# RIVM-bioinformatics/TrueConsense

Measured on AMD Instinct MI355X. Metric: reference positions/sec (BAM file -> consensus FASTA, 1M reads x 29 903 bp per BAM), higher is better.
Workload: dtype int32

## Files before the change

### trueconsense_amd/csrc/bgzf_device.h

```cpp
#pragma once
#include "bgzf_host.h"
#include "tcmi_internal.h"

namespace {

#ifndef TCMI_INFLATE_LL_ROOT
#define TCMI_INFLATE_LL_ROOT 9
#endif
#ifndef TCMI_INFLATE_D_ROOT
#define TCMI_INFLATE_D_ROOT 8
#endif
constexpr int LL_ROOT = TCMI_INFLATE_LL_ROOT, D_ROOT = TCMI_INFLATE_D_ROOT, CL_ROOT = 7;
static_assert(D_ROOT >= CL_ROOT, "the code-length table borrows the distance table's LDS");
constexpr int MAX_REC_PER_BLOCK = 65536 / 36 + 2;

static __constant__ uint8_t CL_ORDER[19] = {16, 17, 18, 0, 8, 7, 9, 6, 10, 5, 11, 4, 12, 3, 13, 2, 14, 1, 15};

__device__ inline uint32_t uni(uint32_t v) { return (uint32_t)__builtin_amdgcn_readfirstlane((int)v); }
__device__ __forceinline__ void wave_sync() { __builtin_amdgcn_fence(__ATOMIC_ACQ_REL, "wavefront"); __builtin_amdgcn_wave_barrier(); }

template <int CTRL, int ROW_MASK>
__device__ __forceinline__ uint32_t dpp_shift(uint32_t v)
{
    return (uint32_t)__builtin_amdgcn_update_dpp(0, (int)v, CTRL, ROW_MASK, 0xF, true);
}
__device__ __forceinline__ uint32_t wave_scan_add(uint32_t v)
{
    v += dpp_shift<0x111, 0xF>(v);
    v += dpp_shift<0x112, 0xF>(v);
    v += dpp_shift<0x114, 0xF>(v);
    v += dpp_shift<0x118, 0xF>(v);
    v += dpp_shift<0x142, 0xA>(v);
    v += dpp_shift<0x143, 0xC>(v);
    return v;
}
__device__ __forceinline__ uint32_t wave_scan_max(uint32_t v)
{
    v = max(v, dpp_shift<0x111, 0xF>(v));
    v = max(v, dpp_shift<0x112, 0xF>(v));
    v = max(v, dpp_shift<0x114, 0xF>(v));
    v = max(v, dpp_shift<0x118, 0xF>(v));
    v = max(v, dpp_shift<0x142, 0xA>(v));
    v = max(v, dpp_shift<0x143, 0xC>(v));
    return v;
}

constexpr uint32_t E_LIT = 1u << 8, E_BASE = 1u << 9, E_EOB = 1u << 10;
enum { K_LITLEN = 0, K_DIST = 1, K_CODELEN = 2 };

typedef uint32_t tab_t;

__device__ inline uint32_t make_entry(int kind, int sym, int nbits)
{
    if (sym < 0) return 0u;
    if (kind == K_CODELEN) return (uint32_t)nbits | ((uint32_t)sym << 16);
    if (kind == K_LITLEN) {
        if (sym < 256) return (uint32_t)nbits | E_LIT | ((uint32_t)sym << 16);
        if (sym == 256) return (uint32_t)nbits | E_EOB;
        const int s = sym - 257;
        if (s > 28) return 0u;
        int eb = 0, base = 3 + s;
        if (s == 28) base = 258;
        else if (s >= 8) { eb = (s >> 2) - 1; base = 3 + ((4 + (s & 3)) << eb); }
        return (uint32_t)nbits | ((uint32_t)(nbits + eb) << 11) | E_BASE | ((uint32_t)eb << 16) | ((uint32_t)base << 20);
    }
    if (sym > 29) return 0u;
    int eb = 0, base = 1 + sym;
    if (sym >= 4) { eb = (sym >> 1) - 1; base = 1 + ((2 + (sym & 1)) << eb); }
    return (uint32_t)nbits | ((uint32_t)eb << 4) | E_BASE | ((uint32_t)base << 16);
}

template <int MAXG, int ROOT>
__device__ __forceinline__ bool build_table(const uint8_t *lens, int n, uint16_t *cnt, uint16_t *sym, tab_t *tab, int kind, uint32_t *rs)
{
    const int lane = threadIdx.x & 63;
    wave_sync();
    int l[MAXG];
#pragma unroll
    for (int g = 0; g < MAXG; ++g) l[g] = g * 64 + lane < n ? (int)lens[g * 64 + lane] : 0;
    int c[16];
#pragma unroll
    for (int len = 0; len < 16; ++len) c[len] = 0;
#pragma unroll
    for (int g = 0; g < MAXG; ++g) {
#pragma unroll
        for (int len = 1; len <= 15; ++len) c[len] += (int)__popcll(__ballot(l[g] == len));
    }
    {
        int mine = 0;
#pragma unroll
        for (int len = 1; len <= 15; ++len) mine = lane == len ? c[len] : mine;
        if (lane < 16) cnt[lane] = (uint16_t)mine;
    }
    int off[16], first[16];
    int left = 1, o = 0, f = 0;
    bool ok = true;
#pragma unroll
    for (int len = 1; len <= 15; ++len) {
        left = (left << 1) - c[len];
        if (left < 0) ok = false;
        off[len] = o;
        first[len] = f;
        o += c[len];
        f = (f + c[len]) << 1;
        if (len == ROOT && lane == 0) { rs[0] = (uint32_t)f; rs[1] = (uint32_t)o; }
    }
    {
        int nx[16];
#pragma unroll
        for (int len = 1; len <= 15; ++len) nx[len] = off[len];
#pragma unroll
        for (int g = 0; g < MAXG; ++g) {
#pragma unroll
            for (int len = 1; len <= 15; ++len) {
                const unsigned long long m = __ballot(l[g] == len);
                if (m) {
                    const int below = (int)__builtin_amdgcn_mbcnt_hi((uint32_t)(m >> 32), __builtin_amdgcn_mbcnt_lo((uint32_t)m, 0u));
                    if (l[g] == len) sym[nx[len] + below] = (uint16_t)(g * 64 + lane);
                    nx[len] += (int)__popcll(m);
                }
            }
        }
    }
    wave_sync();
    for (int i = lane; i < (1 << ROOT); i += 64) {
        const uint32_t r = __builtin_bitreverse32((uint32_t)i) >> (32 - ROOT);
        int L = 0, si = 0;
#pragma unroll
        for (int len = 1; len <= ROOT; ++len) {
            const uint32_t d = (r >> (ROOT - len)) - (uint32_t)first[len];
            const bool hit = d < (uint32_t)c[len];
            L = hit ? len : L;
            si = hit ? off[len] + (int)d : si;
        }
        tab[i] = L ? make_entry(kind, (int)sym[si], L) : 0u;
    }
    wave_sync();
    return uni(ok ? 1u : 0u) != 0;
}

constexpr uint32_t TOK_LIT = 1u << 31, TOK_RAW = 1u << 30;
constexpr uint32_t TOK_LIT2 = 1u << 24;
constexpr uint32_t RAW_PIECE = 8191;

#define TCMI_STAMP(buf_, blk_, k_) do { if (buf_) { if ((threadIdx.x & 63) == 0) (buf_)[(size_t)(blk_) * 16 + (k_)] = __builtin_amdgcn_s_memtime(); } } while (0)
#define TCMI_STAMP_ADD(buf_, blk_, k_, v_) do { if (buf_) { if ((threadIdx.x & 63) == 0) (buf_)[(size_t)(blk_) * 16 + (k_)] += (v_); } } while (0)

}

struct tcmi_bgzf_decode_args {
    const uint8_t *d_file;
    const void *d_desc;
    uint32_t *d_tok;
    uint32_t *d_ntok;
    uint8_t *d_out;
    uint32_t *d_slot;
    uint32_t *d_nrec;
    int32_t *d_over;
    uint32_t *d_first;
    uint32_t *d_stat;
    size_t n_blocks;
    size_t first_block = 0, count = ~(size_t)0;
    uint64_t tok_base = 0;
    uint32_t pay_dwords;
    uint32_t n_ref;
    int verify_crc = 1;
    int scratch_div = 1;
    int short_tokens;
};
int tcmi_bgzf_decode_launch(tcmi_ctx *ctx, const tcmi_bgzf_decode_args &a);
int tcmi_bgzf_symbols_launch(tcmi_ctx *ctx, const tcmi_bgzf_decode_args &a, size_t b_first, size_t nb, uint64_t *stamps, bool report, bool *two_literals);
int tcmi_bgzf_copy_launch(tcmi_ctx *ctx, const tcmi_bgzf_decode_args &a, size_t b_first, size_t nb, uint64_t *stamps, bool report, bool two_literals);
```

### trueconsense_amd/csrc/bgzf_symbols.hip

```cpp
#include <algorithm>
#include <cstdio>
#include <cstdlib>

#include "bgzf_device.h"

namespace {

constexpr int CL_SLAB = 496;
struct BlkTabs {
    tab_t ll[1 << LL_ROOT];
    tab_t dt[1 << D_ROOT];
    tab_t long_ll[288], long_d[32];
    uint32_t lim_ll[16 - LL_ROOT], fb_ll[16 - LL_ROOT], lim_d[16 - D_ROOT], fb_d[16 - D_ROOT];
    uint32_t pos;
    uint32_t end;
    uint32_t ntok;
    uint32_t err;
    uint32_t go;
    uint32_t last;
};
struct HdrScratch {
    uint8_t lens[320];
    uint8_t cll[20];
    uint16_t sym_ll[288], sym_d[32], sym_cl[20];
    uint16_t cnt_ll[16], cnt_d[16], cnt_cl[16];
    uint32_t rs[6];
};
#ifndef TCMI_SYM_MOVE
#define TCMI_SYM_MOVE 8
#endif
#ifndef TCMI_SYM_ROWS
#define TCMI_SYM_ROWS 32
#endif
#ifndef TCMI_SYM_WAVES
#define TCMI_SYM_WAVES 5
#endif
constexpr int RING = 8;
struct PassALds {
    uint2 ring[64][RING];
    uint2 rec[64];
};
template <int NB>
struct SymLds {
    BlkTabs b[NB];
    union {
        HdrScratch h[NB];
        PassALds a;
    };
};
static_assert((CL_SLAB + 16) * 4 <= sizeof(tab_t) * (1 << LL_ROOT), "the code-length position table borrows the literal/length table's LDS");

struct SymArgs {
    const uint32_t *__restrict__ file32;
    const BlockDesc *blocks;
    uint32_t *tokens;
    uint32_t *n_tok;
    uint32_t *status;
    int32_t n_blocks;
    int32_t first_block;
    uint32_t pay_dwords;
    uint32_t win_dwords;
    uint32_t gather_max;
    uint32_t shift_bias;
    uint32_t scratch_div;
    uint64_t *stamps;
};

__device__ __forceinline__ uint32_t peek32(const uint32_t *pay, uint32_t p)
{
    const uint32_t w = p >> 5;
    return __builtin_amdgcn_alignbit(pay[w + 1], pay[w], p);
}
__device__ __forceinline__ void peek64(const uint32_t *pay, uint32_t p, uint32_t &lo, uint32_t &hi)
{
    const uint32_t w = p >> 5;
    const uint32_t w0 = pay[w], w1 = pay[w + 1], w2 = pay[w + 2];
    lo = __builtin_amdgcn_alignbit(w1, w0, p);
    hi = __builtin_amdgcn_alignbit(w2, w1, p);
}

template <int ROOT>
__device__ __forceinline__ void build_long(const uint16_t *cnt, const uint16_t *sym, const uint32_t *rs, int kind, tab_t *out, uint32_t *lim_out,
                                           uint32_t *fb_out)
{
    const int lane = threadIdx.x & 63;
    uint32_t first = uni(rs[0]);
    const uint32_t at = uni(rs[1]);
    uint32_t n = 0;
    uint32_t cs[15 - ROOT];
    uint32_t my_lim = 0x10000u, my_fb = 0;
#pragma unroll
    for (int len = ROOT + 1; len <= 15; ++len) {
        const uint32_t c = uni(cnt[len]);
        cs[len - ROOT - 1] = c;
        if (lane == len - ROOT - 1) { my_lim = (first + c) << (15 - len); my_fb = (first & 0xFFFFu) | (n << 16); }
        first = (first + c) << 1;
        n += c;
    }
    if (lane <= 15 - ROOT) { lim_out[lane] = my_lim; fb_out[lane] = my_fb; }
    for (uint32_t i = (uint32_t)lane; i < n; i += 64) {
        uint32_t base = 0;
        int mylen = 15;
#pragma unroll
        for (int len = ROOT + 1; len <= 15; ++len) {
            const uint32_t c = cs[len - ROOT - 1];
            if (i >= base && i < base + c) mylen = len;
            base += c;
        }
        out[i] = make_entry(kind, (int)sym[at + i], mylen);
    }
}

template <int ROOT>
__device__ __forceinline__ uint32_t long_lookup(const uint32_t *lim, const uint32_t *fb, const tab_t *tab, uint32_t bits)
{
    const uint32_t r15 = __builtin_bitreverse32(bits) >> 17;
    uint32_t n = 0;
#pragma unroll
    for (int k = 0; k < 15 - ROOT; ++k) n += r15 >= lim[k] ? 1u : 0u;
    if (n >= (uint32_t)(15 - ROOT)) return 0u;
    const uint32_t f = fb[n];
    const uint32_t code = r15 >> (14 - ROOT - n);
    if (code < (f & 0xFFFFu)) return 0u;
    return tab[(f >> 16) + (code - (f & 0xFFFFu))];
}

template <int NB>
__device__ __forceinline__ uint32_t group_scan_add(uint32_t v)
{
    v += dpp_shift<0x111, 0xF>(v);
    v += dpp_shift<0x112, 0xF>(v);
    v += dpp_shift<0x114, 0xF>(v);
    v += dpp_shift<0x118, 0xF>(v);
    v += dpp_shift<0x142, 0xA>(v);
    if (NB == 1) v += dpp_shift<0x143, 0xC>(v);
    return v;
}

enum { SY_LIT = 0, SY_MATCH = 1, SY_EOB = 2, SY_BAD = 3 };

__device__ __forceinline__ void block_header(BlkTabs &T, HdrScratch &H, const uint32_t *pay, uint32_t base_bit, uint32_t *toks, uint32_t cap, bool &last,
                                          uint64_t *stamps, int blk, bool one_header = false)
{
    const int lane = threadIdx.x & 63;
    uint32_t pos = uni(T.pos), ntok = uni(T.ntok), err = ST_OK;
    const uint32_t end = uni(T.end);
    bool go = false;
    while (!last && err == ST_OK && !go) {
        if (pos + 3u > end) { err = ST_BAD_STREAM; break; }
        const uint32_t h = uni(peek32(pay, pos));
        last = (h & 1u) != 0;
        const uint32_t type = (h >> 1) & 3u;
        pos += 3;
        if (type == 0) {
            pos = (pos + 7u) & ~7u;
            if (pos + 32u > end) { err = ST_BAD_STREAM; break; }
            const uint32_t v = uni(peek32(pay, pos));
            const uint32_t len = v & 0xFFFFu;
            if (((v >> 16) ^ len) != 0xFFFFu) { err = ST_BAD_STREAM; break; }
            pos += 32;
            if (pos + len * 8u > end) { err = ST_BAD_STREAM; break; }
            const uint32_t off = (pos - base_bit) >> 3;
            const uint32_t pieces = (len + RAW_PIECE - 1u) / RAW_PIECE;
            if (ntok + pieces > cap) { err = ST_BAD_STREAM; break; }
            if ((uint32_t)lane < pieces) {
                const uint32_t o = (uint32_t)lane * RAW_PIECE;
                toks[ntok + (uint32_t)lane] = TOK_RAW | (min(len - o, RAW_PIECE) << 17) | (off + o);
            }
            ntok += pieces;
            pos += len * 8u;
            if (one_header) break;
            continue;
        }
        if (type == 3) { err = ST_BAD_STREAM; break; }
        int nlen = 288, ndist = 32;
        wave_sync();
        if (type == 1) {
            for (int i = lane; i < 320; i += 64) H.lens[i] = i < 144 ? 8 : i < 256 ? 9 : i < 280 ? 7 : i < 288 ? 8 : 5;
        } else {
            if (pos + 14u > end) { err = ST_BAD_STREAM; break; }
            const uint32_t hh = uni(peek32(pay, pos));
            nlen = (int)(hh & 31u) + 257;
            ndist = (int)((hh >> 5) & 31u) + 1;
            const int ncode = (int)((hh >> 10) & 15u) + 4;
            pos += 14;
            if (nlen > 286 || ndist > 30) { err = ST_BAD_STREAM; break; }
            if (lane < 19) H.cll[lane] = 0;
            wave_sync();
            for (int i0 = 0; i0 < ncode; i0 += 8) {
                const uint32_t v = uni(peek32(pay, pos + (uint32_t)i0 * 3u));
                const int k = i0 + lane;
                if (lane < 8 && k < ncode) H.cll[CL_ORDER[k]] = (uint8_t)((v >> (3 * lane)) & 7u);
            }
            pos += (uint32_t)ncode * 3u;
            if (uni(build_table<1, CL_ROOT>(H.cll, 19, H.cnt_cl, H.sym_cl, T.dt, K_CODELEN, H.rs + 4) ? 1u : 0u) == 0u) { err = ST_BAD_STREAM; break; }
            for (int i = lane; i < 320; i += 64) H.lens[i] = 0;
            uint32_t *const P = T.ll;
            uint32_t got = 0, prev = 0;
            const uint32_t total = (uint32_t)(nlen + ndist);
            bool first = true;
            while (got < total && err == ST_OK) {
                wave_sync();
#pragma unroll 2
                for (int o = lane; o < CL_SLAB + 16; o += 64) {
                    const uint32_t v = peek32(pay, pos + (uint32_t)o);
                    const uint32_t e = T.dt[v & ((1u << CL_ROOT) - 1u)];
                    const uint32_t nb = e & 15u, sym = e >> 16;
                    const uint32_t x = v >> nb;
                    const uint32_t eb = sym < 16u ? 0u : sym == 16u ? 2u : sym == 17u ? 3u : 7u;
                    const uint32_t rep = sym < 16u ? 1u : sym == 18u ? 11u + (x & 127u) : 3u + (x & (sym == 16u ? 3u : 7u));
                    const uint32_t val = sym <= 16u ? sym : 0u;
                    P[o] = nb && o < CL_SLAB ? (nb + eb) | (rep << 4) | (val << 12) : 0u;
                }
                wave_sync();
                uint16_t *const J = reinterpret_cast<uint16_t *>(T.long_ll);
                static_assert(sizeof(T.long_ll) >= 512 * sizeof(uint16_t) && CL_SLAB + 16 <= 512, "the doubling table borrows the long-code table's LDS");
#pragma unroll
                for (int i = 0; i < 8; ++i) {
                    const uint32_t at0 = (uint32_t)lane + 64u * i;
                    const uint32_t e0 = at0 < (uint32_t)CL_SLAB + 16u ? P[at0] : 0u;
                    J[at0] = (uint16_t)(e0 ? at0 + (e0 & 15u) : at0);
                }
                wave_sync();
                uint32_t pm[5];
                pm[0] = 0;
#pragma unroll
                for (int k = 0; k < 6; ++k) {
                    if (((uint32_t)lane >> k) & 1u) pm[0] = J[pm[0]];
                    uint32_t t8[8];
#pragma unroll
                    for (int i = 0; i < 8; ++i) t8[i] = J[lane + 64 * i];
#pragma unroll
                    for (int i = 0; i < 8; ++i) t8[i] = J[t8[i]];
                    wave_sync();
#pragma unroll
                    for (int i = 0; i < 8; ++i) J[lane + 64 * i] = (uint16_t)t8[i];
                    wave_sync();
                }
#pragma unroll
                for (int m = 1; m < 5; ++m) pm[m] = J[pm[m - 1]];
                uint32_t o = 0;
                bool stopped = false;
#pragma unroll
                for (int m = 0; m < 5; ++m) {
                    if (!(got < total && err == ST_OK && !stopped)) break;
                    uint32_t mine = P[pm[m]];
                    const unsigned long long zmask = __ballot(mine == 0);
                    const uint32_t nv = zmask ? (uint32_t)__builtin_ctzll(zmask) : 64u;
                    if ((uint32_t)lane >= nv) mine = 0;
                    uint32_t rep = (mine >> 4) & 255u;
                    const uint32_t incl0 = wave_scan_add(rep);
                    const unsigned long long reach = __ballot(mine != 0 && got + incl0 >= total);
                    const uint32_t n_take = reach ? min(nv, (uint32_t)__builtin_ctzll(reach) + 1u) : nv;
                    if ((uint32_t)lane >= n_take) { mine = 0; rep = 0; }
                    const uint32_t v = mine >> 12;
                    const uint32_t at = got + incl0 - ((mine >> 4) & 255u);
                    const uint32_t named = wave_scan_max(mine != 0 && v != 16u ? (uint32_t)lane + 1u : 0u);
                    const uint32_t theirs = (uint32_t)__builtin_amdgcn_ds_bpermute((int)((named - 1u) << 2), (int)v);
                    const uint32_t val = named ? theirs : prev;
                    if (__ballot(mine != 0 && (at + rep > total || (first && lane == 0 && v == 16u)))) { err = ST_BAD_STREAM; break; }
                    if (mine != 0 && val != 0) {
#pragma unroll
                        for (uint32_t i = 0; i < 6; ++i)
                            if (i < rep) H.lens[at + i] = (uint8_t)val;
                    }
                    if (n_take) {
                        prev = (uint32_t)__builtin_amdgcn_readlane((int)val, (int)(n_take - 1u));
                        got += (uint32_t)__builtin_amdgcn_readlane((int)incl0, (int)(n_take - 1u));
                        o = (uint32_t)__builtin_amdgcn_readlane((int)(pm[m] + (mine & 15u)), (int)(n_take - 1u));
                        first = false;
                    }
                    if (n_take < 64u && got < total) {
                        stopped = true;
                        o = (uint32_t)__builtin_amdgcn_readlane((int)pm[m], (int)n_take);
                        if (o < (uint32_t)CL_SLAB) err = ST_BAD_STREAM;
                    }
                }
                if (err == ST_OK && got < total && !stopped) err = ST_BAD_STREAM;
                pos += o;
                if (pos > end) err = ST_BAD_STREAM;
            }
            if (err != ST_OK) break;
            wave_sync();
            if (uni(H.lens[256]) == 0) { err = ST_BAD_STREAM; break; }
        }
        TCMI_STAMP(stamps, blk, 2);
        if (uni(build_table<5, LL_ROOT>(H.lens, nlen, H.cnt_ll, H.sym_ll, T.ll, K_LITLEN, H.rs) ? 1u : 0u) == 0u) { err = ST_BAD_STREAM; break; }
        if (uni(build_table<1, D_ROOT>(H.lens + nlen, ndist, H.cnt_d, H.sym_d, T.dt, K_DIST, H.rs + 2) ? 1u : 0u) == 0u) { err = ST_BAD_STREAM; break; }
        build_long<LL_ROOT>(H.cnt_ll, H.sym_ll, H.rs, K_LITLEN, T.long_ll, T.lim_ll, T.fb_ll);
        build_long<D_ROOT>(H.cnt_d, H.sym_d, H.rs + 2, K_DIST, T.long_d, T.lim_d, T.fb_d);
        if (pos >= end) { err = ST_BAD_STREAM; break; }
        go = true;
        TCMI_STAMP(stamps, blk, 3);
    }
    wave_sync();
    if (lane == 0) { T.pos = pos; T.ntok = ntok; T.err = err; T.go = go && err == ST_OK ? 1u : 0u; T.last = last ? 1u : 0u; }
}

#define TCMI_PAIR_LOOK "v_lshrrev_b32 v44, v50, v47\n" "v_and_b32 v44, 0x1ff, v44\n" "v_lshl_add_u32 v44, v44, 2, %[tabs]\n" "ds_read_b32 v44, v44\n"
#define TCMI_PAIR_RESOLVE "s_waitcnt lgkmcnt(0)\n" "v_and_b32 v40, v49, v44\n" "v_and_b32 v45, 15, v44\n" "v_add_u32 v46, v52, v45\n" "v_xor_b32 v42, %[p], v52\n" "v_lshrrev_b32 v42, %[shift], v42\n" "v_bfe_u32 v40, v40, 8, 1\n" "v_cmp_gt_u32 vcc, 10, v50\n" "v_cmp_eq_u32 s[86:87], 1, v40\n" "s_and_b64 vcc, vcc, s[86:87]\n" "v_cmp_eq_u32 s[86:87], 0, v42\n" "s_and_b64 vcc, vcc, s[86:87]\n" "v_cmp_le_u32 s[86:87], v46, %[wend]\n" "s_and_b64 vcc, vcc, s[86:87]\n" "v_bfe_u32 v40, v44, 16, 8\n" "v_lshl_or_b32 v40, v40, 8, v51\n" "v_or_b32 v40, 0x1000000, v40\n" "v_cndmask_b32 v51, v51, v40, vcc\n" "v_cndmask_b32 v52, v52, v46, vcc\n"
#define TCMI_PASS_A_ASM(PAIR_LOOK_, PAIR_RESOLVE_) \
                asm volatile( \
                    "s_mov_b64 s[92:93], exec\n" \
                    "LT%=:\n" \
                    "s_mov_b64 exec, %[run]\n" \
                    "s_cbranch_execz LX%=\n" \
                    "v_lshrrev_b32 v40, %[shift], %[p]\n" \
                    "v_cmp_ne_u32 vcc, v40, %[kprev]\n" \
                    "s_and_saveexec_b64 s[80:81], vcc\n" \
                    "s_cbranch_execz LA1%=\n" \
                    "v_mov_b32 %[kprev], v40\n" \
                    "v_and_b32 v41, 7, v40\n" \
                    "v_lshl_add_u32 v41, v41, 3, %[ringb]\n" \
                    "ds_write2_b32 v41, %[p], %[total] offset1:1\n" \
                    "v_mov_b32 %[crossp], %[p]\n" \
                    "v_mov_b32 %[crosst], %[total]\n" \
                    "LA1%=:\n" \
                    "s_mov_b64 exec, %[run]\n" \
                    "s_and_b32 s90, %[rounds], 3\n" \
                    "s_cmp_eq_u32 s90, 3\n" \
                    "s_cbranch_scc0 LC%=\n" \
                    "v_cmp_ne_u32 vcc, -1, %[crossp]\n" \
                    "s_and_saveexec_b64 s[80:81], vcc\n" \
                    "s_cbranch_execz LB9%=\n" \
                    "v_add_u32 v41, -1, %[lim]\n" \
                    "v_min_u32 v41, %[tgt], v41\n" \
                    "v_lshl_add_u32 v42, v41, 3, %[recbase]\n" \
                    "ds_read2_b32 v[44:45], v42 offset1:1\n" \
                    "v_lshrrev_b32 v40, %[shift], %[crossp]\n" \
                    "v_and_b32 v40, 7, v40\n" \
                    "v_lshlrev_b32 v40, 3, v40\n" \
                    "s_waitcnt lgkmcnt(0)\n" \
                    "v_and_b32 v43, 3, v44\n" \
                    "v_cmp_ne_u32 vcc, 0, v43\n" \
                    "v_cmp_ge_u32 s[86:87], %[crossp], v45\n" \
                    "s_and_b64 vcc, vcc, s[86:87]\n" \
                    "v_cmp_lt_u32 s[86:87], %[tgt], %[lim]\n" \
                    "s_and_b64 vcc, vcc, s[86:87]\n" \
                    "s_and_saveexec_b64 s[82:83], vcc\n" \
                    "v_cmp_eq_u32 vcc, 1, v43\n" \
                    "v_add_u32 %[tgt], 1, %[tgt]\n" \
                    "s_and_b64 exec, exec, vcc\n" \
                    "v_lshrrev_b32 %[tgt], 8, v44\n" \
                    "s_mov_b64 exec, s[82:83]\n" \
                    "v_cmp_lt_u32 vcc, %[tgt], %[lim]\n" \
                    "s_and_b64 exec, exec, vcc\n" \
                    "s_cbranch_execz LB8%=\n" \
                    "v_lshl_add_u32 v42, %[tgt], 6, v40\n" \
                    "v_add_u32 v42, %[ringbase], v42\n" \
                    "ds_read2_b32 v[44:45], v42 offset1:1\n" \
                    "s_waitcnt lgkmcnt(0)\n" \
                    "v_cmp_eq_u32 vcc, v44, %[crossp]\n" \
                    "s_and_b64 exec, exec, vcc\n" \
                    "s_cbranch_execz LB8%=\n" \
                    "v_mov_b32 %[midx], v45\n" \
                    "v_mov_b32 %[state], 1\n" \
                    "v_mov_b32 %[p], %[crossp]\n" \
                    "v_mov_b32 %[total], %[crosst]\n" \
                    "v_lshl_or_b32 v43, %[tgt], 8, 1\n" \
                    "ds_write2_b32 %[recb], v43, %[p] offset1:1\n" \
                    "s_andn2_b64 %[run], %[run], exec\n" \
                    "LB8%=:\n" \
                    "s_mov_b64 exec, s[80:81]\n" \
                    "v_mov_b32 %[crossp], -1\n" \
                    "LB9%=:\n" \
                    "s_mov_b64 exec, %[run]\n" \
                    "s_cbranch_execz LX%=\n" \
                    "LC%=:\n" \
                    "v_cmp_lt_u32 vcc, %[p], %[wend]\n" \
                    "s_xor_b64 s[86:87], vcc, exec\n" \
                    "s_cmp_lg_u64 s[86:87], 0\n" \
                    "s_cbranch_scc1 LDend%=\n" \
                    "LC1%=:\n" \
                    "v_lshrrev_b32 v40, 5, %[p]\n" \
                    "v_lshl_add_u32 v40, v40, 2, %[pay]\n" \
                    "ds_read2_b32 v[44:45], v40 offset1:1\n" \
                    "ds_read_b32 v46, v40 offset:8\n" \
                    "s_waitcnt lgkmcnt(0)\n" \
                    "v_alignbit_b32 v47, v45, v44, %[p]\n" \
                    "v_alignbit_b32 v48, v46, v45, %[p]\n" \
                    "v_and_b32 v40, 0x1ff, v47\n" \
                    "v_lshl_add_u32 v40, v40, 2, %[tabs]\n" \
                    "ds_read_b32 v49, v40\n" \
                    "s_waitcnt lgkmcnt(0)\n" \
                    "v_and_b32 v50, 15, v49\n" \
                    "v_cmp_eq_u32 vcc, 0, v50\n" \
                    "s_cbranch_vccnz LLl%=\n" \
                    "LC2%=:\n" \
                    "v_bfe_u32 v41, v49, 8, 3\n" \
                    "v_cmp_eq_u32 vcc, 4, v41\n" \
                    "s_cbranch_vccnz LDeob%=\n" \
                    "LC3%=:\n" \
                    "v_bfe_u32 v51, v49, 16, 8\n" \
                    "v_or_b32 v51, 0x80000000, v51\n" \
                    "v_add_u32 v52, %[p], v50\n" \
                    PAIR_LOOK_ \
                    "s_mov_b64 s[88:89], exec\n" \
                    "v_cmp_eq_u32 vcc, 2, v41\n" \
                    "s_and_b64 exec, exec, vcc\n" \
                    "s_cbranch_execz LC5%=\n" \
                    "v_bfe_u32 v53, v49, 11, 5\n" \
                    "v_alignbit_b32 v54, v48, v47, v53\n" \
                    "v_and_b32 v40, 0xff, v54\n" \
                    "v_lshl_add_u32 v40, v40, 2, %[tabs]\n" \
                    "ds_read_b32 v55, v40 offset:%[odt]\n" \
                    "v_lshrrev_b32 v42, v50, v47\n" \
                    "v_bfe_u32 v43, v49, 16, 4\n" \
                    "v_bfe_u32 v42, v42, 0, v43\n" \
                    "v_bfe_u32 v43, v49, 20, 9\n" \
                    "v_add_u32 v56, v43, v42\n" \
                    "s_waitcnt lgkmcnt(0)\n" \
                    "v_and_b32 v57, 15, v55\n" \
                    "v_cmp_eq_u32 vcc, 0, v57\n" \
                    "s_cbranch_vccnz LLd%=\n" \
                    "LC4%=:\n" \
                    "v_bfe_u32 v43, v55, 4, 4\n" \
                    "v_lshrrev_b32 v42, v57, v54\n" \
                    "v_bfe_u32 v42, v42, 0, v43\n" \
                    "v_lshrrev_b32 v40, 16, v55\n" \
                    "v_add_u32 v42, v42, v40\n" \
                    "v_add_u32 v42, -1, v42\n" \
                    "v_lshl_or_b32 v51, v42, 9, v56\n" \
                    "v_add3_u32 v52, %[p], v53, v57\n" \
                    "v_add_u32 v52, v52, v43\n" \
                    "LC5%=:\n" \
                    "s_and_b64 exec, s[88:89], %[run]\n" \
                    "s_cbranch_execz LT%=\n" \
                    PAIR_RESOLVE_ \
                    "v_mov_b32 %[p], v52\n" \
                    "v_cmp_gt_u32 vcc, %[p], %[end]\n" \
                    "s_cbranch_vccnz LDover%=\n" \
                    "LC6%=:\n" \
                    "s_mov_b64 s[80:81], exec\n" \
                    "v_cmp_ne_u32 vcc, 0, %[room]\n" \
                    "s_and_b64 exec, exec, vcc\n" \
                    "global_store_dword %[sptr], v51, off\n" \
                    "v_add_u32 %[room], -1, %[room]\n" \
                    "v_lshl_add_u64 %[sptr], %[sptr], 0, %[sstride]\n" \
                    "s_mov_b64 exec, s[80:81]\n" \
                    "v_add_u32 %[total], 1, %[total]\n" \
                    "s_add_u32 %[rounds], %[rounds], 1\n" \
                    "s_branch LT%=\n" \
                    "LDend%=:\n" \
                    "s_mov_b64 s[82:83], exec\n" \
                    "s_mov_b64 exec, s[86:87]\n" \
                    "v_mov_b32 %[state], 3\n" \
                    "v_mov_b32 v43, 3\n" \
                    "ds_write2_b32 %[recb], v43, %[p] offset1:1\n" \
                    "s_andn2_b64 %[run], %[run], exec\n" \
                    "s_andn2_b64 exec, s[82:83], s[86:87]\n" \
                    "s_cbranch_execz LT%=\n" \
                    "s_branch LC1%=\n" \
                    "LDeob%=:\n" \
                    "s_mov_b64 s[82:83], exec\n" \
                    "s_and_b64 exec, exec, vcc\n" \
                    "v_add_u32 %[p], %[p], v50\n" \
                    "v_add_u32 %[total], 1, %[total]\n" \
                    "v_mov_b32 %[state], 2\n" \
                    "v_mov_b32 v43, 2\n" \
                    "ds_write2_b32 %[recb], v43, %[p] offset1:1\n" \
                    "s_andn2_b64 %[run], %[run], exec\n" \
                    "s_andn2_b64 exec, s[82:83], exec\n" \
                    "s_cbranch_execz LT%=\n" \
                    "s_branch LC3%=\n" \
                    "LDover%=:\n" \
                    "s_mov_b64 s[82:83], exec\n" \
                    "s_and_b64 exec, exec, vcc\n" \
                    "v_mov_b32 %[state], 3\n" \
                    "v_mov_b32 v43, 3\n" \
                    "ds_write2_b32 %[recb], v43, %[p] offset1:1\n" \
                    "s_andn2_b64 %[run], %[run], exec\n" \
                    "s_andn2_b64 exec, s[82:83], exec\n" \
                    "s_cbranch_execz LT%=\n" \
                    "s_branch LC6%=\n" \
                    "LLl%=:\n" \
                    "s_mov_b64 s[84:85], exec\n" \
                    "s_and_b64 exec, exec, vcc\n" \
                    "v_bfrev_b32 v40, v47\n" \
                    "v_lshrrev_b32 v40, 17, v40\n" \
                    "v_add_u32 v41, %[oliml], %[tabs]\n" \
                    "ds_read2_b32 v[58:59], v41 offset1:1\n" \
                    "ds_read2_b32 v[60:61], v41 offset0:2 offset1:3\n" \
                    "ds_read2_b32 v[62:63], v41 offset0:4 offset1:5\n" \
                    "s_waitcnt lgkmcnt(0)\n" \
                    "v_sub_u32 v58, v40, v58\n" \
                    "v_sub_u32 v59, v40, v59\n" \
                    "v_sub_u32 v60, v40, v60\n" \
                    "v_sub_u32 v61, v40, v61\n" \
                    "v_sub_u32 v62, v40, v62\n" \
                    "v_sub_u32 v63, v40, v63\n" \
                    "v_ashrrev_i32 v58, 31, v58\n" \
                    "v_ashrrev_i32 v59, 31, v59\n" \
                    "v_ashrrev_i32 v60, 31, v60\n" \
                    "v_ashrrev_i32 v61, 31, v61\n" \
                    "v_ashrrev_i32 v62, 31, v62\n" \
                    "v_ashrrev_i32 v63, 31, v63\n" \
                    "v_add3_u32 v58, v58, v59, v60\n" \
                    "v_add3_u32 v61, v61, v62, v63\n" \
                    "v_add3_u32 v42, v58, v61, 6\n" \
                    "v_min_u32 v41, 5, v42\n" \
                    "v_lshl_add_u32 v41, v41, 2, %[tabs]\n" \
                    "ds_read_b32 v43, v41 offset:%[ofbll]\n" \
                    "v_sub_u32 v41, 5, v42\n" \
                    "v_lshrrev_b32 v41, v41, v40\n" \
                    "s_waitcnt lgkmcnt(0)\n" \
                    "v_and_b32 v40, 0xffff, v43\n" \
                    "v_cmp_ge_u32 vcc, v41, v40\n" \
                    "v_cmp_gt_u32 s[86:87], 6, v42\n" \
                    "s_and_b64 vcc, vcc, s[86:87]\n" \
                    "v_sub_u32 v41, v41, v40\n" \
                    "v_lshrrev_b32 v40, 16, v43\n" \
                    "v_add_u32 v41, v41, v40\n" \
                    "v_and_b32 v41, 0x1ff, v41\n" \
                    "v_lshl_add_u32 v41, v41, 2, %[tabs]\n" \
                    "ds_read_b32 v49, v41 offset:%[olongll]\n" \
                    "s_waitcnt lgkmcnt(0)\n" \
                    "v_and_b32 v50, 15, v49\n" \
                    "v_cmp_ne_u32 s[86:87], 0, v50\n" \
                    "s_and_b64 vcc, vcc, s[86:87]\n" \
                    "s_andn2_b64 exec, exec, vcc\n" \
                    "s_cbranch_execz LLl9%=\n" \
                    "v_mov_b32 %[state], 3\n" \
                    "v_mov_b32 v43, 3\n" \
                    "ds_write2_b32 %[recb], v43, %[p] offset1:1\n" \
                    "s_andn2_b64 %[run], %[run], exec\n" \
                    "LLl9%=:\n" \
                    "s_and_b64 exec, s[84:85], %[run]\n" \
                    "s_cbranch_execz LT%=\n" \
                    "s_branch LC2%=\n" \
                    "LLd%=:\n" \
                    "s_mov_b64 s[84:85], exec\n" \
                    "s_and_b64 exec, exec, vcc\n" \
                    "v_bfrev_b32 v40, v54\n" \
                    "v_lshrrev_b32 v40, 17, v40\n" \
                    "v_add_u32 v41, %[olimd], %[tabs]\n" \
                    "ds_read2_b32 v[58:59], v41 offset1:1\n" \
                    "ds_read2_b32 v[60:61], v41 offset0:2 offset1:3\n" \
                    "ds_read2_b32 v[62:63], v41 offset0:4 offset1:5\n" \
                    "ds_read_b32 v42, v41 offset:24\n" \
                    "s_waitcnt lgkmcnt(0)\n" \
                    "v_sub_u32 v58, v40, v58\n" \
                    "v_sub_u32 v59, v40, v59\n" \
                    "v_sub_u32 v60, v40, v60\n" \
                    "v_sub_u32 v61, v40, v61\n" \
                    "v_sub_u32 v62, v40, v62\n" \
                    "v_sub_u32 v63, v40, v63\n" \
                    "v_sub_u32 v42, v40, v42\n" \
                    "v_ashrrev_i32 v58, 31, v58\n" \
                    "v_ashrrev_i32 v59, 31, v59\n" \
                    "v_ashrrev_i32 v60, 31, v60\n" \
                    "v_ashrrev_i32 v61, 31, v61\n" \
                    "v_ashrrev_i32 v62, 31, v62\n" \
                    "v_ashrrev_i32 v63, 31, v63\n" \
                    "v_ashrrev_i32 v42, 31, v42\n" \
                    "v_add3_u32 v58, v58, v59, v60\n" \
                    "v_add3_u32 v61, v61, v62, v63\n" \
                    "v_add3_u32 v42, v58, v61, v42\n" \
                    "v_add_u32 v42, 7, v42\n" \
                    "v_min_u32 v41, 6, v42\n" \
                    "v_lshl_add_u32 v41, v41, 2, %[tabs]\n" \
                    "ds_read_b32 v43, v41 offset:%[ofbd]\n" \
                    "v_sub_u32 v41, 6, v42\n" \
                    "v_lshrrev_b32 v41, v41, v40\n" \
                    "s_waitcnt lgkmcnt(0)\n" \
                    "v_and_b32 v40, 0xffff, v43\n" \
                    "v_cmp_ge_u32 vcc, v41, v40\n" \
                    "v_cmp_gt_u32 s[86:87], 7, v42\n" \
                    "s_and_b64 vcc, vcc, s[86:87]\n" \
                    "v_sub_u32 v41, v41, v40\n" \
                    "v_lshrrev_b32 v40, 16, v43\n" \
                    "v_add_u32 v41, v41, v40\n" \
                    "v_and_b32 v41, 31, v41\n" \
                    "v_lshl_add_u32 v41, v41, 2, %[tabs]\n" \
                    "ds_read_b32 v55, v41 offset:%[olongd]\n" \
                    "s_waitcnt lgkmcnt(0)\n" \
                    "v_and_b32 v57, 15, v55\n" \
                    "v_cmp_ne_u32 s[86:87], 0, v57\n" \
                    "s_and_b64 vcc, vcc, s[86:87]\n" \
                    "s_andn2_b64 exec, exec, vcc\n" \
                    "s_cbranch_execz LLd9%=\n" \
                    "v_mov_b32 %[state], 3\n" \
                    "v_mov_b32 v43, 3\n" \
                    "ds_write2_b32 %[recb], v43, %[p] offset1:1\n" \
                    "s_andn2_b64 %[run], %[run], exec\n" \
                    "LLd9%=:\n" \
                    "s_and_b64 exec, s[84:85], %[run]\n" \
                    "s_cbranch_execz LC5%=\n" \
                    "s_branch LC4%=\n" \
                    "LX%=:\n" \
                    "s_mov_b64 exec, s[92:93]\n" \
                    : [p] "+v"(p), [total] "+v"(total), [tgt] "+v"(tgt_abs), [midx] "+v"(midx), [kprev] "+v"(kprev), [state] "+v"(state), \
                      [room] "+v"(room), [crossp] "+v"(crossp), [crosst] "+v"(crosst), [sptr] "+v"(sptr), [run] "+s"(run), [rounds] "+s"(rounds) \
                    : [tabs] "v"(tabs), [pay] "v"(payb), [end] "v"(b_end), [wend] "v"(b_soft), [shift] "v"(shift), [ringb] "v"(ringb), [recb] "v"(recb), [lim] "v"(lim), \
// ... 311 lines not shown
```

Baseline: 71.77 million.

## Rebuild Huffman tables with radix ranking and key-propagated slot fill

Per-block Huffman table construction in the symbols kernel changes approach. Code lengths are ranked with a 4-bit ballot radix trick instead of 15 ballots per length. Per-length limits come from a DPP row scan instead of a serial loop. Root-table slots are filled by writing a start key per length and propagating it with a wave max-scan, replacing the per-slot loop over all lengths. Entries are precomputed per symbol into the long tables, so build_long now just compacts the long-code entries. This is meant to cut the header-decode cost per BGZF block, but it adds LDS traffic and syncs and is subtle encoding logic that could hide correctness bugs.

```diff
diff --git a/trueconsense_amd/csrc/bgzf_device.h b/trueconsense_amd/csrc/bgzf_device.h
--- a/trueconsense_amd/csrc/bgzf_device.h
+++ b/trueconsense_amd/csrc/bgzf_device.h
@@ -1,5 +1,6 @@
 #pragma once
 #include "bgzf_host.h"
+#include "huffman_rule.h"
 #include "tcmi_internal.h"
 
 namespace {
@@ -45,98 +46,97 @@
     return v;
 }
 
-constexpr uint32_t E_LIT = 1u << 8, E_BASE = 1u << 9, E_EOB = 1u << 10;
-enum { K_LITLEN = 0, K_DIST = 1, K_CODELEN = 2 };
+constexpr uint32_t E_LIT = TCMI_HUFF_E_LIT, E_BASE = TCMI_HUFF_E_BASE, E_EOB = TCMI_HUFF_E_EOB;
+enum { K_LITLEN = TCMI_HUFF_LITLEN, K_DIST = TCMI_HUFF_DIST, K_CODELEN = TCMI_HUFF_CODELEN };
 
 typedef uint32_t tab_t;
 
-__device__ inline uint32_t make_entry(int kind, int sym, int nbits)
+__device__ inline uint32_t make_entry(int kind, int sym, int nbits) { return tcmi_huff_entry(kind, sym, nbits); }
+
+__device__ __forceinline__ uint32_t row_scan_add(uint32_t v)
 {
-    if (sym < 0) return 0u;
-    if (kind == K_CODELEN) return (uint32_t)nbits | ((uint32_t)sym << 16);
-    if (kind == K_LITLEN) {
-        if (sym < 256) return (uint32_t)nbits | E_LIT | ((uint32_t)sym << 16);
-        if (sym == 256) return (uint32_t)nbits | E_EOB;
-        const int s = sym - 257;
-        if (s > 28) return 0u;
-        int eb = 0, base = 3 + s;
-        if (s == 28) base = 258;
-        else if (s >= 8) { eb = (s >> 2) - 1; base = 3 + ((4 + (s & 3)) << eb); }
-        return (uint32_t)nbits | ((uint32_t)(nbits + eb) << 11) | E_BASE | ((uint32_t)eb << 16) | ((uint32_t)base << 20);
-    }
-    if (sym > 29) return 0u;
-    int eb = 0, base = 1 + sym;
-    if (sym >= 4) { eb = (sym >> 1) - 1; base = 1 + ((2 + (sym & 1)) << eb); }
-    return (uint32_t)nbits | ((uint32_t)eb << 4) | E_BASE | ((uint32_t)base << 16);
+    v += dpp_shift<0x111, 0xF>(v);
+    v += dpp_shift<0x112, 0xF>(v);
+    v += dpp_shift<0x114, 0xF>(v);
+    v += dpp_shift<0x118, 0xF>(v);
+    return v;
 }
 
 template <int MAXG, int ROOT>
-__device__ __forceinline__ bool build_table(const uint8_t *lens, int n, uint16_t *cnt, uint16_t *sym, tab_t *tab, int kind, uint32_t *rs)
+__device__ __forceinline__ bool build_table(const uint8_t *lens, int n, uint16_t *cnt, uint16_t *sym, tab_t *ent, uint32_t *ol, tab_t *tab, int kind, uint32_t *rs)
 {
-    const int lane = threadIdx.x & 63;
+    static_assert(ROOT >= 7 && ROOT <= 14, "a turn of the slot loop is 64 slots");
+    int lane = threadIdx.x & 63;
+    asm volatile("" : "+v"(lane));
     wave_sync();
-    int l[MAXG];
+    uint32_t lp[MAXG];
 #pragma unroll
-    for (int g = 0; g < MAXG; ++g) l[g] = g * 64 + lane < n ? (int)lens[g * 64 + lane] : 0;
-    int c[16];
-#pragma unroll
-    for (int len = 0; len < 16; ++len) c[len] = 0;
+    for (int g = 0; g < MAXG; ++g) lp[g] = g * 64 + lane < n ? (uint32_t)lens[g * 64 + lane] & 15u : 0u;
+    if (lane < 16) ol[lane] = 0;
+    wave_sync();
 #pragma unroll
     for (int g = 0; g < MAXG; ++g) {
+        const uint32_t len = lp[g];
+        uint32_t eq_lo = ~0u, eq_hi = ~0u;
 #pragma unroll
-        for (int len = 1; len <= 15; ++len) c[len] += (int)__popcll(__ballot(l[g] == len));
+        for (int k = 0; k < 4; ++k) {
+            const uint32_t mine = (uint32_t)((int32_t)(len << (31 - k)) >> 31);
+            const unsigned long long m = __ballot(mine != 0);
+            eq_lo &= ~((uint32_t)m ^ mine);
+            eq_hi &= ~((uint32_t)(m >> 32) ^ mine);
+        }
+        const uint32_t below = __builtin_amdgcn_mbcnt_hi(eq_hi, __builtin_amdgcn_mbcnt_lo(eq_lo, 0u));
+        const uint32_t before = ol[len];
+        lp[g] = len | ((before + below) << 4);
+        asm volatile("" : "+v"(lp[g]));
+        wave_sync();
+        ol[len] = before + (uint32_t)__popc(eq_lo) + (uint32_t)__popc(eq_hi);
+        wave_sync();
     }
+    const uint32_t c = lane >= 1 && lane < 16 ? ol[lane] : 0u;
+    const uint32_t term = tcmi_huff_term(c, lane & 15);
+    const uint32_t o_incl = row_scan_add(c), lim15 = row_scan_add(term);
+    constexpr int S = 1 << (ROOT - 6);
+    uint32_t *const mine = tab + lane * S;
+#pragma unroll
+    for (int j = 0; j < S; ++j) mine[j] = 0u;
+    wave_sync();
+    if (lane < 16) {
+        cnt[lane] = (uint16_t)c;
+        ol[lane] = o_incl - c;
+    }
+    if (lane == ROOT) { rs[0] = lim15 >> (14 - ROOT); rs[1] = o_incl; }
     {
-        int mine = 0;
+        const uint32_t start = tcmi_huff_key_start(lim15 - term, ROOT);
+        if (lane >= 1 && lane <= ROOT + 1 && (c != 0 || lane == ROOT + 1) && start < (1u << ROOT)) tab[start] = tcmi_huff_key(lane & 15, o_incl - c, lim15 - term, ROOT);
+    }
+    const bool ok = tcmi_huff_fits((uint32_t)__builtin_amdgcn_readlane((int)lim15, 15));
+    wave_sync();
 #pragma unroll
-        for (int len = 1; len <= 15; ++len) mine = lane == len ? c[len] : mine;
-        if (lane < 16) cnt[lane] = (uint16_t)mine;
-    }
-    int off[16], first[16];
-    int left = 1, o = 0, f = 0;
-    bool ok = true;
-#pragma unroll
-    for (int len = 1; len <= 15; ++len) {
-        left = (left << 1) - c[len];
-        if (left < 0) ok = false;
-        off[len] = o;
-        first[len] = f;
-        o += c[len];
-        f = (f + c[len]) << 1;
-        if (len == ROOT && lane == 0) { rs[0] = (uint32_t)f; rs[1] = (uint32_t)o; }
-    }
-    {
-        int nx[16];
-#pragma unroll
-        for (int len = 1; len <= 15; ++len) nx[len] = off[len];
-#pragma unroll
-        for (int g = 0; g < MAXG; ++g) {
-#pragma unroll
-            for (int len = 1; len <= 15; ++len) {
-                const unsigned long long m = __ballot(l[g] == len);
-                if (m) {
-                    const int below = (int)__builtin_amdgcn_mbcnt_hi((uint32_t)(m >> 32), __builtin_amdgcn_mbcnt_lo((uint32_t)m, 0u));
-                    if (l[g] == len) sym[nx[len] + below] = (uint16_t)(g * 64 + lane);
-                    nx[len] += (int)__popcll(m);
-                }
-            }
+    for (int g = 0; g < MAXG; ++g) {
+        const uint32_t len = lp[g] & 15u;
+        if (len) {
+            const uint32_t at = ol[len] + (lp[g] >> 4);
+            sym[at] = (uint16_t)(g * 64 + lane);
+            ent[at] = make_entry(kind, g * 64 + lane, (int)len);
         }
     }
+    uint32_t key[S];
+#pragma unroll
+    for (int j = 0; j < S; ++j) key[j] = mine[j];
+#pragma unroll
+    for (int j = 1; j < S; ++j) key[j] = max(key[j], key[j - 1]);
+    const uint32_t in_front = dpp_shift<0x138, 0xF>(wave_scan_max(key[S - 1]));
     wave_sync();
-    for (int i = lane; i < (1 << ROOT); i += 64) {
-        const uint32_t r = __builtin_bitreverse32((uint32_t)i) >> (32 - ROOT);
-        int L = 0, si = 0;
+    const uint32_t i0 = __builtin_bitreverse32((uint32_t)lane) >> 26;
 #pragma unroll
-        for (int len = 1; len <= ROOT; ++len) {
-            const uint32_t d = (r >> (ROOT - len)) - (uint32_t)first[len];
-            const bool hit = d < (uint32_t)c[len];
-            L = hit ? len : L;
-            si = hit ? off[len] + (int)d : si;
-        }
-        tab[i] = L ? make_entry(kind, (int)sym[si], L) : 0u;
+    for (int j = 0; j < S; ++j) {
+        const uint32_t k = max(key[j], in_front);
+        const uint32_t e = ent[tcmi_huff_key_index(k, (uint32_t)(lane * S + j))];
+        tab[i0 + 64u * (__builtin_bitreverse32((uint32_t)j) >> (38 - ROOT))] = tcmi_huff_key_filled(k, ROOT) ? e : 0u;
     }
     wave_sync();
-    return uni(ok ? 1u : 0u) != 0;
+    return ok;
 }
 
 constexpr uint32_t TOK_LIT = 1u << 31, TOK_RAW = 1u << 30;
diff --git a/trueconsense_amd/csrc/bgzf_symbols.hip b/trueconsense_amd/csrc/bgzf_symbols.hip
--- a/trueconsense_amd/csrc/bgzf_symbols.hip
+++ b/trueconsense_amd/csrc/bgzf_symbols.hip
@@ -25,6 +25,7 @@
     uint16_t sym_ll[288], sym_d[32], sym_cl[20];
     uint16_t cnt_ll[16], cnt_d[16], cnt_cl[16];
     uint32_t rs[6];
+    uint32_t ol[16];
 };
 #ifndef TCMI_SYM_MOVE
 #define TCMI_SYM_MOVE 8
@@ -80,34 +81,29 @@
 }
 
 template <int ROOT>
-__device__ __forceinline__ void build_long(const uint16_t *cnt, const uint16_t *sym, const uint32_t *rs, int kind, tab_t *out, uint32_t *lim_out,
-                                           uint32_t *fb_out)
+__device__ __forceinline__ void build_long(const uint16_t *cnt, const uint32_t *rs, tab_t *out, uint32_t *lim_out, uint32_t *fb_out)
 {
     const int lane = threadIdx.x & 63;
     uint32_t first = uni(rs[0]);
     const uint32_t at = uni(rs[1]);
     uint32_t n = 0;
-    uint32_t cs[15 - ROOT];
     uint32_t my_lim = 0x10000u, my_fb = 0;
 #pragma unroll
     for (int len = ROOT + 1; len <= 15; ++len) {
         const uint32_t c = uni(cnt[len]);
-        cs[len - ROOT - 1] = c;
         if (lane == len - ROOT - 1) { my_lim = (first + c) << (15 - len); my_fb = (first & 0xFFFFu) | (n << 16); }
         first = (first + c) << 1;
         n += c;
     }
     if (lane <= 15 - ROOT) { lim_out[lane] = my_lim; fb_out[lane] = my_fb; }
-    for (uint32_t i = (uint32_t)lane; i < n; i += 64) {
-        uint32_t base = 0;
-        int mylen = 15;
-#pragma unroll
-        for (int len = ROOT + 1; len <= 15; ++len) {
-            const uint32_t c = cs[len - ROOT - 1];
-            if (i >= base && i < base + c) mylen = len;
-            base += c;
-        }
-        out[i] = make_entry(kind, (int)sym[at + i], mylen);
+    if (at == 0) return;
+    for (uint32_t i0 = 0; i0 < n; i0 += 64) {
+        const uint32_t i = i0 + (uint32_t)lane;
+        uint32_t e = 0;
+        if (i < n) e = out[at + i];
+        wave_sync();
+        if (i < n) out[i] = e;
+        wave_sync();
     }
 }
 
@@ -193,7 +189,7 @@
                 if (lane < 8 && k < ncode) H.cll[CL_ORDER[k]] = (uint8_t)((v >> (3 * lane)) & 7u);
             }
             pos += (uint32_t)ncode * 3u;
-            if (uni(build_table<1, CL_ROOT>(H.cll, 19, H.cnt_cl, H.sym_cl, T.dt, K_CODELEN, H.rs + 4) ? 1u : 0u) == 0u) { err = ST_BAD_STREAM; break; }
+            if (!build_table<1, CL_ROOT>(H.cll, 19, H.cnt_cl, H.sym_cl, T.long_d, H.ol, T.dt, K_CODELEN, H.rs + 4)) { err = ST_BAD_STREAM; break; }
             for (int i = lane; i < 320; i += 64) H.lens[i] = 0;
             uint32_t *const P = T.ll;
             uint32_t got = 0, prev = 0;
@@ -285,10 +281,11 @@
             if (uni(H.lens[256]) == 0) { err = ST_BAD_STREAM; break; }
         }
         TCMI_STAMP(stamps, blk, 2);
-        if (uni(build_table<5, LL_ROOT>(H.lens, nlen, H.cnt_ll, H.sym_ll, T.ll, K_LITLEN, H.rs) ? 1u : 0u) == 0u) { err = ST_BAD_STREAM; break; }
-        if (uni(build_table<1, D_ROOT>(H.lens + nlen, ndist, H.cnt_d, H.sym_d, T.dt, K_DIST, H.rs + 2) ? 1u : 0u) == 0u) { err = ST_BAD_STREAM; break; }
-        build_long<LL_ROOT>(H.cnt_ll, H.sym_ll, H.rs, K_LITLEN, T.long_ll, T.lim_ll, T.fb_ll);
-        build_long<D_ROOT>(H.cnt_d, H.sym_d, H.rs + 2, K_DIST, T.long_d, T.lim_d, T.fb_d);
+        static_assert(sizeof(T.long_ll) >= 288 * sizeof(tab_t) && sizeof(T.long_d) >= 32 * sizeof(tab_t), "an entry per symbol");
+        if (!build_table<5, LL_ROOT>(H.lens, nlen, H.cnt_ll, H.sym_ll, T.long_ll, H.ol, T.ll, K_LITLEN, H.rs)) { err = ST_BAD_STREAM; break; }
+        if (!build_table<1, D_ROOT>(H.lens + nlen, ndist, H.cnt_d, H.sym_d, T.long_d, H.ol, T.dt, K_DIST, H.rs + 2)) { err = ST_BAD_STREAM; break; }
+        build_long<LL_ROOT>(H.cnt_ll, H.rs, T.long_ll, T.lim_ll, T.fb_ll);
+        build_long<D_ROOT>(H.cnt_d, H.rs + 2, T.long_d, T.lim_d, T.fb_d);
         if (pos >= end) { err = ST_BAD_STREAM; break; }
         go = true;
         TCMI_STAMP(stamps, blk, 3);
diff --git a/trueconsense_amd/csrc/huffman_rule.h b/trueconsense_amd/csrc/huffman_rule.h
--- /dev/null
+++ b/trueconsense_amd/csrc/huffman_rule.h
@@ -0,0 +1,62 @@
+#pragma once
+#include <stdint.h>
+
+#if defined(__HIP__)
+#define TCMI_HUFF_HD __attribute__((host)) __attribute__((device))
+#else
+#define TCMI_HUFF_HD
+#endif
+
+enum { TCMI_HUFF_LITLEN = 0, TCMI_HUFF_DIST = 1, TCMI_HUFF_CODELEN = 2 };
+enum { TCMI_HUFF_E_LIT = 1 << 8, TCMI_HUFF_E_BASE = 1 << 9, TCMI_HUFF_E_EOB = 1 << 10 };
+
+TCMI_HUFF_HD inline uint32_t tcmi_huff_term(uint32_t cnt, int len) { return cnt << (15 - len); }
+TCMI_HUFF_HD inline bool tcmi_huff_fits(uint32_t lim15_of_15) { return lim15_of_15 <= (1u << 15); }
+TCMI_HUFF_HD inline uint32_t tcmi_huff_root_limit(uint32_t lim15, int root) { return lim15 >> (15 - root); }
+TCMI_HUFF_HD inline uint32_t tcmi_huff_key(int L, uint32_t off, uint32_t lim15_before, int root)
+{
+    if (L > root) return ((uint32_t)L << 27) | (512u << 5) | 31u;
+    return ((uint32_t)L << 27) | (((off + 512u - (lim15_before >> (15 - L))) & 0x3FFFFFu) << 5) | (uint32_t)(root - L);
+}
+TCMI_HUFF_HD inline uint32_t tcmi_huff_key_start(uint32_t lim15_before, int root) { return tcmi_huff_root_limit(lim15_before, root); }
+TCMI_HUFF_HD inline uint32_t tcmi_huff_key_index(uint32_t key, uint32_t r) { return (r >> (key & 31u)) + ((key >> 5) & 0x3FFFFFu) - 512u; }
+TCMI_HUFF_HD inline bool tcmi_huff_key_filled(uint32_t key, int root) { return key < ((uint32_t)(root + 1) << 27); }
+
+TCMI_HUFF_HD inline void tcmi_huff_limits(const uint32_t cnt[16], uint32_t lim15[16], uint32_t off[16])
+{
+    uint32_t lim = 0, o = 0;
+    lim15[0] = 0;
+    off[0] = 0;
+    for (int len = 1; len <= 15; ++len) {
+        off[len] = o;
+        o += cnt[len];
+        lim += tcmi_huff_term(cnt[len], len);
+        lim15[len] = lim;
+    }
+}
+TCMI_HUFF_HD inline int tcmi_huff_slot_length(uint32_t r, const uint32_t lim15[16], int root)
+{
+    int L = 1;
+    for (int len = 1; len <= root; ++len) L += r >= tcmi_huff_root_limit(lim15[len], root) ? 1 : 0;
+    return L;
+}
+
+TCMI_HUFF_HD inline uint32_t tcmi_huff_entry(int kind, int sym, int nbits)
+{
+    if (sym < 0) return 0u;
+    if (kind == TCMI_HUFF_CODELEN) return (uint32_t)nbits | ((uint32_t)sym << 16);
+    if (kind == TCMI_HUFF_LITLEN) {
+        if (sym < 256) return (uint32_t)nbits | TCMI_HUFF_E_LIT | ((uint32_t)sym << 16);
+        if (sym == 256) return (uint32_t)nbits | TCMI_HUFF_E_EOB;
+        const int s = sym - 257;
+        if (s > 28) return 0u;
+        int eb = 0, base = 3 + s;
+        if (s == 28) base = 258;
+        else if (s >= 8) { eb = (s >> 2) - 1; base = 3 + ((4 + (s & 3)) << eb); }
+        return (uint32_t)nbits | ((uint32_t)(nbits + eb) << 11) | TCMI_HUFF_E_BASE | ((uint32_t)eb << 16) | ((uint32_t)base << 20);
+    }
+    if (sym > 29) return 0u;
+    int eb = 0, base = 1 + sym;
+    if (sym >= 4) { eb = (sym >> 1) - 1; base = 1 + ((2 + (sym & 1)) << eb); }
+    return (uint32_t)nbits | ((uint32_t)eb << 4) | TCMI_HUFF_E_BASE | ((uint32_t)base << 16);
+}
```

After: 74.41 million, median of 6. +3.7%, better.
